# bastienjacquet/CudaDepthMapIntegration

Measured on AMD Instinct MI355X. Metric: Gvoxel-projections/s, higher is better.
Workload: dtype f64

## Files before the change

### cudadepthmapintegration_amd/build.py

```python
from __future__ import annotations

import os
import re
import shutil
import subprocess
from concurrent.futures import ThreadPoolExecutor

_HERE = os.path.dirname(os.path.abspath(__file__))
ROOT = os.path.dirname(_HERE)
CSRC = os.path.join(_HERE, "csrc")
OBJ_DIR = os.path.join(ROOT, "build", "obj")
LIB_PATH = os.path.join(CSRC, "libdmi_hip.so")

SOURCES = ["fusion_kernels.hip", "fusion_tile.hip", "fusion_classify.hip", "coloration_kernels.hip", "mesh_depth_render.hip", "grid_post.hip", "point_smooth.hip", "isosurface.hip", "isosurface_components.hip", "isosurface_smooth.hip", "isosurface_decimate.hip", "isosurface_holes.hip", "isosurface_support.hip", "depth_consistency.hip", "depth_speckle.hip", "scene_bounds.hip", "dmi_capi.hip", "dmi_capi_views.hip", "dmi_capi_fuse.hip", "dmi_capi_mesh.hip", "dmi_capi_color.hip", "dmi_capi_consistency.hip", "dmi_capi_speckle.hip", "dmi_capi_bounds.hip", "dmi_multi.hip", "host/recon_host.cpp", "host/vti_reader.cpp", "host/vtp_reader.cpp", "host/recon_cli.cpp", "host/color_cli.cpp", "host/dmi_host_capi.cpp"]
HEADERS = ["fusion_kernels.h", "view_records.h", "fusion_launch_rules.h", "fusion_device.h", "dmi_buffer.h", "dmi_context.h", "dmi_color_context.h", "coloration_kernels.h", "mesh_depth_render.h", "depth_consistency.h", "depth_speckle.h", "depth_speckle_rules.h", "union_find_device.h", "scene_bounds.h", "scene_bounds_rules.h", "point_smooth_rules.h", "rounded_quotient.h", "fusion_tile_acc.inc", "isosurface_table.inc", os.path.join("host", "recon_host.h"),
           os.path.join("host", "vtk_xml_data.h"), os.path.join("host", "vti_reader.h"), os.path.join("host", "vtp_reader.h"),
           os.path.join("host", "recon_cli.h"), os.path.join("host", "color_cli.h"), os.path.join("host", "fan_triangulate.h"),
           os.path.join("..", "..", "include", "dmi.h"), os.path.join("..", "..", "include", "dmi_host.h")]
CLI_MAINS = ["recon_cli_main.cpp", "color_cli_main.cpp"]

COMMON_FLAGS = ["-O3", "-std=c++17", "-fPIC", "-ffp-contract=off", "-fno-fast-math", "-Wall", "-Wno-unused-function",
                "-Wno-inline-asm", "-Wno-pass-failed"]
HIP_FLAGS = ["--offload-arch=gfx950", "-mllvm", "-disable-promote-alloca-to-vector", "-Xoffload-linker", "--discard-all"]
OPTIONAL_LLVM_FLAGS = ["-amdgpu-use-amdgpu-trackers=1"]


def _probe_llvm_flag(flag: str) -> bool:
    import tempfile
# ... 178 lines not shown
    for m in re.finditer(r"\.amdhsa_kernel (_ZN3dmi\S*fuse_tile_kernel\S*)\b(.*?)\.end_amdhsa_kernel", asm_text, re.S):
        size = re.search(r"\.amdhsa_private_segment_fixed_size (\d+)", m.group(2))
        out[m.group(1)] = int(size.group(1)) if size else 0
    return out


def lds_sizes(asm_text: str) -> dict:
    out = {}
    for m in re.finditer(r"\.amdhsa_kernel (_ZN3dmi\S*fuse_tile_kernel\S*)\b(.*?)\.end_amdhsa_kernel", asm_text, re.S):
        size = re.search(r"\.amdhsa_group_segment_fixed_size (\d+)", m.group(2))
        out[m.group(1)] = int(size.group(1)) if size else 0
    return out


def wait_state_counts(asm_text: str) -> dict:
    import re

    out = {}
    for m in re.finditer(r"^(_ZN3dmi\S*fuse_tile_kernel\S*):.*?\.end_amdhsa_kernel", asm_text, re.S | re.M):
        out[m.group(1)] = len(re.findall(r"^\s*s_nop\b", m.group(0), re.M))
    return out


def _audit_digest() -> str:
    return source_digest([os.path.join(CSRC, "fusion_tile.hip")] + _headers())


def audit_is_current() -> bool:
    import json

    marker = os.path.join(OBJ_DIR, "acc_audit.json")
    try:
        with open(marker) as fh:
            return json.load(fh).get("digest") == _audit_digest()
    except (OSError, ValueError):
        return False


def run_accumulator_audit(verbose: bool = False) -> int:
    import json
    import tempfile

    hipcc = hipcc_path()
    with tempfile.TemporaryDirectory() as tmp:
        out = os.path.join(tmp, "fusion_tile.s")
        cmd = [hipcc] + COMMON_FLAGS + HIP_FLAGS + ["--cuda-device-only", "-S", os.path.join(CSRC, "fusion_tile.hip"), "-o", out]
# ... 7 lines not shown
    nops = wait_state_counts(text)
    lds = lds_sizes(text)
    table = {}
    for name, size in scratch.items():
        m = re.search(r"fuse_tile_kernelI(\w)(\w)Li(\d+)ELi(\d)ELi(\d)ELi(\d)ELi(\d)ELb([01])ELb([01])ELb([01])ELb([01])ELb([01])(?:ELb([01]))?E", name)
        if not m:
            continue
        depth, grid, tk, wx, wy, minw, group, count, rot, genk, stay, win, zf = m.groups()
        key = f"depth={depth} grid={grid} tk={tk} waves={wx}x{wy} count={count} rot={rot} genk={genk} stay={stay} win={win} zf={zf or 0}"
        production = depth == "f" and count == "0" and genk == "0" and wx == "1" and wy == "1"
        limit = None if not production else ((16 if "-DDMI_TUNING" in COMMON_FLAGS else 0) if tk == "16" else 48)
        table[key] = {"scratch_bytes_per_lane": size, "production": production, "limit": limit, "s_nop": nops.get(name),
                      "lds_bytes_per_workgroup": lds.get(name, 0)}
        if limit is not None and size > limit:
            bad.append(f"{name}: {size} bytes of scratch memory per lane in a production instantiation (limit {limit})")
        waves_per_cu = 4 * (4 if tk == "16" else 5)
        if production and lds.get(name, 0) * waves_per_cu > 160 * 1024:
            bad.append(f"{name}: {lds[name]} bytes of LDS per one-wave workgroup: {waves_per_cu} of them do not fit a CU's 160 KB")
    if bad:
        raise RuntimeError("accumulator-register audit of fusion_tile.hip FAILED (a toolchain change broke the hidden "
                           "register file; results would be silently wrong):\n  " + "\n  ".join(bad[:20]))
    version = subprocess.run([hipcc, "--version"], capture_output=True, text=True).stdout.strip().splitlines()
    os.makedirs(OBJ_DIR, exist_ok=True)
    with open(os.path.join(OBJ_DIR, "acc_audit.json"), "w") as fh:
        json.dump({"instantiations": checked, "violations": 0, "hipcc": version[:2], "digest": _audit_digest(),
                   "scratch_bytes_per_lane": {"max": max(scratch.values()) if scratch else None,
                                              "instantiations_with_scratch": sum(1 for v in scratch.values() if v),
                                              "production_max": max([v["scratch_bytes_per_lane"] for v in table.values() if v["production"]] or [0])},
                   "instantiation_table": table}, fh, indent=1)
    if verbose:
        print(f"accumulator audit: {checked} fuse_tile_kernel instantiations clean ({version[0] if version else 'hipcc'})", flush=True)
    return checked


def _record(mode: str) -> None:
    import json
    import time

    try:
        os.makedirs(OBJ_DIR, exist_ok=True)
        with open(os.path.join(OBJ_DIR, "build_record.json"), "w") as fh:
            json.dump({"mode": mode, "library": os.path.relpath(LIB_PATH, ROOT), "digest": source_digest(), "time": time.time(),
                       "flags": COMMON_FLAGS + HIP_FLAGS}, fh)
    except OSError:
        pass


def build(force: bool = False, verbose: bool = False) -> str:
    if not force and not needs_build():
        _record("up_to_date: the library's digest file names the present sources and flags; nothing compiled")
        return LIB_PATH
    hipcc = hipcc_path()
    os.makedirs(OBJ_DIR, exist_ok=True)
    headers = _headers()
    digest = source_digest()
    if not force and os.path.exists(LIB_PATH) and os.path.exists(_digest_path()):
        srcs = [os.path.join(CSRC, s) for s in _sources()]
        if not any(_stale(_obj(s), [p] + headers) for s, p in zip(_sources(), srcs)):
            force = True

    def compile_one(src: str):
        path = os.path.join(CSRC, src)
        obj = _obj(src)
        if not force and not _stale(obj, [path] + headers):
            return
        cmd = [hipcc] + COMMON_FLAGS + (HIP_FLAGS if src.endswith(".hip") else []) + ["-c", path, "-o", obj]
        if verbose:
            print(" ".join(cmd), flush=True)
        subprocess.check_call(cmd)

    def audit_if_needed(_):
        if force or not audit_is_current():
            run_accumulator_audit(verbose)

    with ThreadPoolExecutor(max_workers=4) as ex:
        jobs = [ex.submit(compile_one, s) for s in _sources()] + [ex.submit(audit_if_needed, None)]
        for j in jobs:
            j.result()
    staged = os.path.join(OBJ_DIR, os.path.basename(LIB_PATH) + f".{os.getpid()}.tmp")
    cmd = [hipcc, "--offload-arch=gfx950", "-shared", "-fPIC"] + [_obj(s) for s in _sources()] + ["-lz", "-ldl", "-pthread", "-o", staged]
    if verbose:
        print(" ".join(cmd), flush=True)
    subprocess.check_call(cmd)
    os.replace(staged, LIB_PATH)
    with open(_digest_path(), "w") as fh:
        fh.write(digest + "\n")
    build_cli(verbose)
    build_color_cli(verbose)
    _record("rebuilt: hipcc compiled the stale objects and linked the library")
    return LIB_PATH


CLI_PATH = os.path.join(CSRC, "dmi_reconstruction")
COLOR_CLI_PATH = os.path.join(CSRC, "dmi_coloration")


def _link_tool(main_src: str, exe: str, verbose: bool) -> str:
    if os.path.basename(LIB_PATH) != "libdmi_hip.so" or LIB_OVERRIDE:
        return ""
# ... 26 lines not shown
```

### cudadepthmapintegration_amd/capi.py

```python
from __future__ import annotations

import ctypes
import os
import sys
from typing import NamedTuple

import numpy as np

from . import build as _build
from .scene import GridDesc, RayPotential, Views

DMI_OK = 0
DMI_F32, DMI_F64 = 0, 1
DMI_DEPTH_AUTO, DMI_DEPTH_F32, DMI_DEPTH_F64 = 0, 1, 2
DMI_COMPONENTS_MIN_TRIANGLES, DMI_COMPONENTS_LARGEST = 0, 1

VARIANT_EXACT_DIVISION = 1
VARIANT_GENERAL_K = 2
VARIANT_FORCE_GENERAL = 16
VARIANT_NO_BRICK_CLASSES = 256
VARIANT_KEEP_BEHIND_ADDS = 1024
VARIANT_NO_INTERIOR = 2048
VARIANT_XCD_RUNS = 8192
VARIANT_ZMAJOR_SLOTS = 16384
VARIANT_PERSISTENT_ALWAYS = 32768
VARIANT_PERSISTENT_NEVER = 65536
VARIANT_NO_WINDOWS = 262144
VARIANT_WINDOWS_ALWAYS = 524288
VARIANT_COST_ORDER = 1048576
VARIANT_NO_COST_ORDER = 2097152
VARIANT_BRICK_CLASSES_ALWAYS = 131072
VARIANT_FIXED_TILE_SHAPE = 4096
VARIANT_SPATIAL_ORDER = 512
VARIANT_TILE_SHAPE = {"tk16_w5_g8_1x1": 0, "tk8_w6_g8_2x2": 32, "tk16_w5_g8_2x2": 64, "tk8_w6": 96, "tk8_w7_g8": 128, "tk16_w5_g4": 160,
                      "tk16_w6_g2": 192, "tk8_w6_g8_1x1": 224}


class GridDescC(ctypes.Structure):
    _fields_ = [("cell_dims", ctypes.c_int32 * 3), ("origin", ctypes.c_double * 3),
                ("spacing", ctypes.c_double * 3), ("grid_matrix", ctypes.c_double * 16)]


class RayPotentialC(ctypes.Structure):
    _fields_ = [("thickness", ctypes.c_double), ("rho", ctypes.c_double), ("eta", ctypes.c_double),
                ("delta", ctypes.c_double)]


class OptionsC(ctypes.Structure):
    _fields_ = [("device", ctypes.c_int32), ("grid_dtype", ctypes.c_int32), ("depth_storage", ctypes.c_int32),
                ("count_hits", ctypes.c_int32), ("kernel_variant", ctypes.c_int32), ("z_first", ctypes.c_int32),
                ("stream", ctypes.c_void_p), ("external_grid", ctypes.c_void_p)]


# ... 1559 lines not shown
```

### cudadepthmapintegration_amd/csrc/dmi_capi_fuse.hip

```cpp
#include "dmi_context.h"

#include <algorithm>
#include <cmath>
#include <cstdlib>
#include <cstring>

using dmi::drain_events;
using dmi::EventPair;
using dmi::fail;
using dmi::flush_zero_fill;
using dmi::FuseArgs;
using dmi::FuseConfig;
using dmi::guarded;
using dmi::MapRec;
using dmi::TileArgs;
using dmi::TileMapRec;

namespace {

int sync_maps(dmi_context *ctx) {
  dmi_context::Views &v = ctx->views;
  const size_t n = v.h_maps.size();
  const size_t cap = std::max<size_t>(64, n * 2);
  bool fresh = false;
// ... 142 lines not shown
  if (!whole_grid) {
    t.sbz_first = a.k_first / (2 * sh.tk);
    t.super_z = (a.k_first + a.k_count + 2 * sh.tk - 1) / (2 * sh.tk) - t.sbz_first;
  }
  if (t.bricks_x > 2047 || t.bricks_y > 2047 || t.bricks_z > 1023)
    return fail(ctx, DMI_ERR_INVALID_ARGUMENT, "dmi_fuse: more bricks along an axis than the tiled kernel's order entries hold");
  t.slot_base = t.sbz_first * t.super_x * t.super_y * 32;
  t.slot_count = t.super_x * t.super_y * t.super_z * 32;
  const int rc = slot_permutation(ctx, t.super_x, t.super_y, t.super_z, (cfg.variant & dmi::VAR_ZMAJOR_SLOTS) != 0, &t.sb_perm);
  if (rc != DMI_OK) return rc;
  t.xcd_run_wg = 32 * std::max(1, t.super_x * t.super_y);
  if (((int64_t)t.super_x * t.super_y * t.super_z * 32 + 16 * (int64_t)t.xcd_run_wg + 64) > (int64_t)0x7fffffff)
    return fail(ctx, DMI_ERR_INVALID_ARGUMENT, "dmi_fuse: grid too large for one launch");
  t.depth_bytes = (int32_t)((int64_t)a.W * a.H * (ctx->views.depth_f64 ? 8 : 4));
  t.kz0 = a.kz0;
  t.ox = a.ox; t.oy = a.oy; t.oz = a.oz; t.sx = a.sx; t.sy = a.sy; t.sz = a.sz;
  std::memcpy(t.g, a.g, sizeof(t.g));
  t.thick = a.thick; t.delta = a.delta; t.rho_pos = a.rho_pos; t.rho_neg = a.rho_neg;
  t.slope = a.slope; t.free_space = a.free_space;
  t.tile_maps = ctx->views.tile_maps.as<TileMapRec>();
  t.grid = a.grid; t.voxel_hits = a.voxel_hits; t.map_hits = a.map_hits;
  t.rotated = dmi::grid_axis_aligned(ctx->grid) ? 0 : 1;
  t.flags = ((cfg.variant & dmi::VAR_NO_INTERIOR) ? dmi::TILE_FLAG_NO_INTERIOR : 0) |
            ((cfg.variant & dmi::VAR_XCD_RUNS) ? dmi::TILE_FLAG_XCD_RUNS : 0);
  t.maps = ctx->views.maps.as<MapRec>();
  t.wbricks_x = (a.nx + 7) / 8;
  t.wbricks_y = (a.ny + 7) / 8;
  return DMI_OK;
}

int cz_table(dmi_context *ctx, const FuseArgs &a, TileArgs *t) {
  const size_t table_doubles = std::max<size_t>(ctx->views.h_maps.size(), 4) * (size_t)t->kpad;
  const size_t need = table_doubles + (size_t)dmi::kFreeSumsMax + 1;
  const int rc = dmi::ensure_idle_buffer(ctx, ctx->tables.cz_table, need * 8, need * 2 * 8);
  if (rc != DMI_OK) return rc;
  t->cz_table = ctx->tables.cz_table.as<double>();
  if (!a.init_from_grid && !ctx->opt.count_hits && a.n_maps <= dmi::kFreeSumsMax) t->free_sums = t->cz_table + table_doubles;
  return DMI_OK;
}

int zero_row(dmi_context *ctx, TileArgs *t) {
  bool fresh = false;
  const int rc = dmi::ensure_idle_buffer(ctx, ctx->tables.zero_row, (uint64_t)t->class_pitch, (uint64_t)t->class_pitch, &fresh);
  if (rc != DMI_OK) return rc;
  if (fresh) DMI_HIP(ctx, hipMemsetAsync(ctx->tables.zero_row.ptr, dmi::BRICK_MIXED, (size_t)t->class_pitch, ctx->stream));
  t->classes = ctx->tables.zero_row.as<uint8_t>();
  t->class_pitch = 0;
// ... 300 lines not shown
```

### cudadepthmapintegration_amd/csrc/fusion_classify.hip

```cpp
#include <algorithm>
#include <cstring>

#include <stdlib.h>

#include "fusion_kernels.h"
#include "fusion_device.h"

namespace dmi {

namespace {

template <typename T>
__device__ __forceinline__ T cload(const T *p) {
  return *reinterpret_cast<const T __attribute__((address_space(4))) *>(reinterpret_cast<uintptr_t>(p));
}

__device__ __forceinline__ float float_below(double d) {
  float f = (float)d;
  if ((double)f > d) f = nextafterf(f, -__builtin_inff());
  return f;
}
__device__ __forceinline__ float float_above(double d) {
  float f = (float)d;
  if ((double)f < d) f = nextafterf(f, __builtin_inff());
// ... 409 lines not shown
  } else if (fp.partial) {
    cls = border_class<GK>(a, fp, pyramid_query<5>(maps[m].pyramid, P, fp.x0, fp.x1, fp.y0, fp.y1));
  }
  const bool inherit_mixed = cls == (uint8_t)(BRICK_MIXED | (MIXED_FREE_OR_NODEPTH << 2)) && speckled;
  coarse[(int64_t)((cbz * cy_n + cby) * cx_n + cbx) * a.class_pitch + m] = inherit_mixed ? (uint8_t)(cls | COARSE_CHILDREN_WRITTEN) : cls;
  if ((cls & 3) == BRICK_MIXED && !inherit_mixed) return;
  for (int dz = 0; dz < per_z; ++dz) {
    const int bz = bz0 + dz;
    if (bz >= bz_first + bz_count) break;
    for (int dy = 0; dy < 4; ++dy) {
      const int by = cby * 4 + dy;
      if (by >= a.wbricks_y) break;
      for (int dx = 0; dx < 4; ++dx) {
        const int bx = cbx * 4 + dx;
        if (bx >= a.wbricks_x) break;
        classes[(int64_t)((bz * a.wbricks_y + by) * a.wbricks_x + bx) * a.class_pitch + m] = cls;
      }
    }
  }
}

constexpr int kWindow = 16;

template <int kQueryTiles, int kChildren, bool ROT, bool GK>
__global__ __launch_bounds__(256) void classify_kernel(const TileArgs a, const MapRec *__restrict__ maps,
                                                       const PyramidDesc P, int tk, uint8_t *__restrict__ classes,
                                                       const uint8_t *__restrict__ coarse, int group_views) {
  constexpr int children = kChildren;
  constexpr int views_per_wave = 64 / children;
  constexpr int per_z = children / 16;
  __shared__ float2 window_mm[4 * views_per_wave][kWindow * kWindow];
  __shared__ uint8_t window_fl[4 * views_per_wave][kWindow * kWindow];
  const int bz_first = 2 * a.sbz_first;
  const int bz_count = min(2 * a.super_z, a.bricks_z - bz_first);
  const int cx_n = (a.wbricks_x + 3) / 4, cy_n = (a.wbricks_y + 3) / 4;
  const int lane = threadIdx.x & 63, wave = __builtin_amdgcn_readfirstlane(threadIdx.x >> 6);
  const int local = blockIdx.x;
  const int cbx = local % cx_n;
  const int ct = local / cx_n;
  const int cby = ct % cy_n, cbz = ct / cy_n + bz_first / per_z;
  const int chunk0 = blockIdx.y * group_views;
  const uint8_t *__restrict__ crow = coarse + (int64_t)((cbz * cy_n + cby) * cx_n + cbx) * a.class_pitch + a.first_map + chunk0;
  const unsigned long long unproven = __builtin_amdgcn_ballot_w64(
      lane < group_views && chunk0 + lane < a.n_maps && (crow[lane] & (3 | COARSE_CHILDREN_WRITTEN)) == BRICK_MIXED);
  if (unproven == 0) return;
  unsigned long long items = views_per_wave == 1 ? unproven & (0x1111111111111111ull << wave)
                                                 : (unproven | (unproven >> 1)) & (0x0101010101010101ull << (2 * wave));
  const int child = lane % children;
  const int bx = cbx * 4 + (child & 3), by = cby * 4 + ((child >> 2) & 3), bz = cbz * per_z + (child >> 4);
  const bool in_grid = bx < a.wbricks_x && by < a.wbricks_y && bz < bz_first + bz_count;
  uint8_t *__restrict__ out = classes + (int64_t)((bz * a.wbricks_y + by) * a.wbricks_x + bx) * a.class_pitch;
  while (items) {
    const int first = __builtin_ctzll(items);
    items &= items - 1;
    const int rel = first + lane / children;
    const int mm = chunk0 + rel;
    const int m = a.first_map + min(mm, a.n_maps - 1);
    const bool mine = in_grid && ((unproven >> rel) & 1ull);
    const MapRec *__restrict__ mr = maps + m;
    BoxFootprint fp;
    fp.query = false;
    fp.partial = false;
    fp.in_margin = false;
    fp.cls = BRICK_SKIP;
// ... 60 lines not shown
            TileAcc d;
            for (int ty = ty0; ty <= ty1; ++ty)
              for (int tx = tx0; tx <= tx1; ++tx) {
                const int w = (ty - wy0) * kWindow + (tx - wx0);
                const float2 mm = win_mm[w];
                d.add_tile(DepthTile{mm.x, mm.y, (uint32_t)win_fl[w], 0u});
              }
            cls = fp.partial ? border_class<GK>(a, fp, d) : class_from_bounds(a, d, fp.czmin, fp.czmax);
            from_window = true;
          }
          __builtin_amdgcn_fence(__ATOMIC_RELEASE, "wavefront");
          __builtin_amdgcn_wave_barrier();
        }
      }
    }
    if (query && !from_window) {
      const TileAcc d = pyramid_query<kQueryTiles>(mr->pyramid, P, fp.x0, fp.x1, fp.y0, fp.y1);
      cls = fp.partial ? border_class<GK>(a, fp, d) : class_from_bounds(a, d, fp.czmin, fp.czmax);
    }
    if (mine) out[m] = cls;
  }
}

constexpr int kOriginViews = 8;
#ifdef DMI_WINPAIR_BRICK_MAJOR
constexpr int kOriginBricks = 256, kOriginWaveSets = 1, kOriginAlign = 4;
#else
constexpr int kOriginBricks = 64, kOriginWaveSets = 4, kOriginAlign = kWinPairBlockViews;
static_assert(kOriginViews * kOriginWaveSets == kWinPairBlockViews, "a workgroup's views are one block of the pair table");
#endif
constexpr uint32_t kNotWanted = 0xfffffffeu;
template <bool ROT>
__global__ __launch_bounds__(256) void window_origin_kernel(const TileArgs a, const MapRec *__restrict__ maps, int tk,
                                                            uint8_t *__restrict__ classes, WinPair *__restrict__ origins,
                                                            int group_views) {
  __shared__ WinPair tile[kOriginViews * kOriginWaveSets][kOriginBricks + 1];
#ifdef DMI_WINPAIR_BRICK_MAJOR
  __shared__ int64_t rows[256];
#endif
  const int bz_first = 2 * a.sbz_first;
  const int bz_count = min(2 * a.super_z, a.bricks_z - bz_first);
  const int64_t n_bricks = (int64_t)a.wbricks_x * a.wbricks_y * bz_count;
  const int lane = threadIdx.x & 63;
  const int tb = threadIdx.x % kOriginBricks;
  const int wset = kOriginWaveSets > 1 ? __builtin_amdgcn_readfirstlane(threadIdx.x / kOriginBricks) : 0;
  const int64_t local = (int64_t)blockIdx.x * kOriginBricks + tb;
  const bool exists = local < n_bricks;
  const int bx = (int)(local % a.wbricks_x);
  const int64_t t = local / a.wbricks_x;
  const int by = (int)(t % a.wbricks_y), bz = (int)(t / a.wbricks_y) + bz_first;
  const int64_t row = (((int64_t)bz * a.wbricks_y + by) * a.wbricks_x + bx) * a.class_pitch;
  const bool eligible = exists && bz * tk + tk <= a.nz;
  (void)lane;
  double wxa, wya, wza;
  {
    const double gx = a.ox + (bx * 8 + 0.5) * a.sx;
    const double gy = a.oy + (by * 8 + 0.5) * a.sy;
    const double gz = a.oz + ((bz * tk + a.kz0) + 0.5) * a.sz;
    wxa = row4(a.g + 0, gx, gy, gz), wya = row4(a.g + 4, gx, gy, gz), wza = row4(a.g + 8, gx, gy, gz);
  }
  const int m_begin = a.first_map, m_end = a.first_map + a.n_maps;
  const int g_wg = (m_begin & ~(kOriginAlign - 1)) + blockIdx.y * (group_views * kOriginWaveSets);
  const int slot0 = wset * group_views;
  const int g_lo = g_wg + slot0;
#ifdef DMI_WINPAIR_BRICK_MAJOR
  rows[threadIdx.x] = row;
#endif
  uint32_t held[kOriginViews / 4];
#pragma unroll
  for (int g = 0; g < kOriginViews / 4; ++g) {
    const int m4 = g_lo + 4 * g;
    held[g] = (eligible && 4 * g < group_views && m4 < m_end) ? *reinterpret_cast<const uint32_t *>(classes + row + m4) : 0u;
    if (4 * g < group_views) {
#pragma unroll
      for (int q = 0; q < 4; ++q) tile[slot0 + 4 * g + q][tb].origin = kNotWanted;
    }
  }
#pragma unroll
  for (int g = 0; g < kOriginViews / 4; ++g) {
    const int m4 = g_lo + 4 * g;
    if (4 * g >= group_views || m4 >= m_end) break;
    const uint32_t c4 = held[g];
#pragma unroll 1
    for (int q = 0; q < 4; ++q) {
      const int m = m4 + q;
      const uint8_t c = (uint8_t)(c4 >> (8 * q));
      const bool want = eligible && m >= m_begin && m < m_end && (c & 0x1f) == (uint8_t)(BRICK_MIXED | (MIXED_FREE_OR_NODEPTH << 2));
      if (__builtin_amdgcn_ballot_w64(want) == 0) continue;
      WinPair wp;
      wp.origin = kNotWanted;
      wp.ax = wp.ay = wp.acz = 0.f;
      if (cload(&a.win_recs[m].e_abs) < __builtin_inff()) {
        const MapRec *src = maps + m;
        const TileMapRec *tsrc = a.tile_maps + m;
        const FootRec *fr = a.foot_recs + m;
        const float(*scp)[4] = tk == 16 ? fr->s16 : fr->s8;
        if (want) {
          const double cza = ((cload(&src->rt[8]) * wxa + cload(&src->rt[9]) * wya) + cload(&src->rt[10]) * wza) + cload(&src->rt[11]);
          const double hxa = __builtin_fma(cload(&tsrc->cpx), wxa, __builtin_fma(cload(&tsrc->cpy), wya, __builtin_fma(cload(&tsrc->cpz), wza, cload(&tsrc->cp0))));
          const double hya = __builtin_fma(cload(&tsrc->cqx), wxa, __builtin_fma(cload(&tsrc->cqy), wya, __builtin_fma(cload(&tsrc->cqz), wza, cload(&tsrc->cq0))));
          const float hx0 = (float)hxa, hy0 = (float)hya, z0 = (float)cza;
          float umin = __builtin_inff(), umax = -__builtin_inff(), vmin = __builtin_inff(), vmax = -__builtin_inff();
// ... 15 lines not shown
            const int cxc = a.W / 2, cyc = a.H / 2;
            const int x0 = (int)__builtin_ceilf(umin - 0.5f - e) + cxc, x1 = (int)__builtin_floorf(umax + 0.5f + e) + cxc;
            const int y0 = (int)__builtin_ceilf(vmin - 0.5f - e) + cyc, y1 = (int)__builtin_floorf(vmax + 0.5f + e) + cyc;
            if (x0 >= -kValidMargin && y0 >= -kValidMargin && x1 < a.W + kValidMargin && y1 < a.H + kValidMargin &&
                x1 - x0 < kWindowCols && y1 - y0 < kWindowRows) {
              wp.origin = (uint32_t)(x0 + kValidMargin) | ((uint32_t)(y0 + kValidMargin) << 16);
              wp.ax = (float)(hxa - (double)(x0 + kWinAnchorX - cxc) * cza);
              wp.ay = (float)(hya - (double)(y0 + kWinAnchorY - cyc) * cza);
              wp.acz = z0;
            }
          }
        }
      }
      if (want) {
        if (wp.origin != kNotWanted)
          tile[slot0 + 4 * g + q][tb] = wp;
        else
          classes[row + m] = (uint8_t)(c | CLASS_NO_WINDOW);
      }
    }
  }
  __syncthreads();
#ifdef DMI_WINPAIR_BRICK_MAJOR
  const int v = threadIdx.x & (kOriginViews - 1);
  const int m = g_lo + v;
  if (v < group_views && m < m_end) {
#pragma unroll
    for (int it = 0; it < 8; ++it) {
      const int b = (threadIdx.x >> 3) + 32 * it;
      const WinPair wp = tile[v][b];
      if (wp.origin != kNotWanted) origins[rows[b] + m] = wp;
    }
  }
#else
  const int wg_views = group_views * kOriginWaveSets;
  const int lg = 31 - __builtin_clz((unsigned)wg_views);
  const int64_t brick0 = (int64_t)blockIdx.x * kOriginBricks + (int64_t)bz_first * a.wbricks_y * a.wbricks_x;
  for (int e = threadIdx.x; e < kOriginBricks * wg_views; e += 256) {
    const int b = e >> lg, v = e & (wg_views - 1);
    const int m = g_wg + v;
    if (m >= m_end) continue;
    const WinPair wp = tile[v][b];
    if (wp.origin != kNotWanted) origins[win_pair_index(brick0 + b, m, a.n_class_bricks)] = wp;
  }
#endif
}


__device__ __forceinline__ bool slot_to_brick(const TileArgs &a, int slot, int &bx, int &by, int &bz) {
  const int within = slot & 31;
  const int code = a.sb_perm[(slot - a.slot_base) >> 5];
  const int sbx = code & 1023, sby = (code >> 10) & 1023, sbz = (code >> 20) + a.sbz_first;
  bx = sbx * 4 + (within & 3);
  by = sby * 4 + ((within >> 2) & 3);
  bz = sbz * 2 + (within >> 4);
  return bx < a.bricks_x && by < a.bricks_y && bz < a.bricks_z;
}

constexpr int kWorkLevels = 4;

__global__ __launch_bounds__(256) void brick_work_kernel(const TileArgs a, int wx, int wy, int n_slots,
// ... 290 lines not shown
      DMI_UPLOAD(double, float);
  } else {
    if (out_is_f64)
      DMI_UPLOAD(float, double);
    else
      DMI_UPLOAD(float, float);
  }
#undef DMI_UPLOAD
  return hipGetLastError();
}

hipError_t launch_build_pyramid_levels(int64_t n_maps, const PyramidDesc &P, DepthTile *pyramids, hipStream_t stream) {
  if (n_maps <= 0 || P.n_levels <= 1) return hipSuccess;
  hipLaunchKernelGGL(pyramid_levels_kernel, dim3((unsigned)n_maps), dim3(1024), 0, stream, P, pyramids);
  return hipGetLastError();
}

hipError_t launch_window_origins(const TileArgs &a, const MapRec *maps_dev, int tk, uint8_t *classes, int general_k,
                                 hipStream_t stream) {
  if (general_k || !a.win_origin || a.n_maps <= 0) return hipSuccess;
  const int bz_count = std::min(2 * a.super_z, a.bricks_z - 2 * a.sbz_first);
  const int64_t n_bricks = (int64_t)a.wbricks_x * a.wbricks_y * bz_count;
  if (n_bricks <= 0) return hipSuccess;
  const int64_t brick_groups = (n_bricks + kOriginBricks - 1) / kOriginBricks;
  const int span = a.first_map + a.n_maps - (a.first_map & ~(kOriginAlign - 1));
  int group_views = kOriginViews;
  const auto view_groups = [&](int gv) { return (span + gv * kOriginWaveSets - 1) / (gv * kOriginWaveSets); };
  while (group_views > 4 && brick_groups * view_groups(group_views) < 2048) group_views >>= 1;
  if (brick_groups > (int64_t)0x7fffffff || a.n_class_bricks > (int64_t)0x7fffffff) return hipErrorInvalidConfiguration;
  const dim3 grid((unsigned)brick_groups, (unsigned)view_groups(group_views));
  if (a.rotated)
    hipLaunchKernelGGL((window_origin_kernel<true>), grid, dim3(256), 0, stream, a, maps_dev, tk, classes, a.win_origin, group_views);
  else
    hipLaunchKernelGGL((window_origin_kernel<false>), grid, dim3(256), 0, stream, a, maps_dev, tk, classes, a.win_origin, group_views);
  return hipGetLastError();
}

hipError_t launch_classify_bricks(const TileArgs &a, const MapRec *maps_dev, const PyramidDesc &P, int tk, uint8_t *classes,
                                  uint8_t *coarse, int general_k, hipStream_t stream) {
  const int bz_count = std::min(2 * a.super_z, a.bricks_z - 2 * a.sbz_first);
  const int64_t n_bricks = (int64_t)a.wbricks_x * a.wbricks_y * bz_count;
  if (n_bricks <= 0 || a.n_maps <= 0) return hipSuccess;
  if (n_bricks > (int64_t)0x7fffffff || (a.n_maps + 3) / 4 > 65535) return hipErrorInvalidConfiguration;
  const int per_z = 32 / tk;
  const int64_t n_boxes = (int64_t)((a.wbricks_x + 3) / 4) * ((a.wbricks_y + 3) / 4) * ((bz_count + per_z - 1) / per_z);
  const dim3 coarse_grid((unsigned)((n_boxes + 3) / 4), (unsigned)((a.n_maps + 63) / 64));
#define DMI_LAUNCH_COARSE(R, G) \
  hipLaunchKernelGGL((classify_coarse_kernel<R, G>), coarse_grid, dim3(64, 4), 0, stream, a, maps_dev, P, tk, classes, coarse)
  if (a.rotated && general_k)
    DMI_LAUNCH_COARSE(true, true);
  else if (a.rotated)
    DMI_LAUNCH_COARSE(true, false);
  else if (general_k)
    DMI_LAUNCH_COARSE(false, true);
  else
    DMI_LAUNCH_COARSE(false, false);
#undef DMI_LAUNCH_COARSE
  hipError_t e = hipGetLastError();
  if (e != hipSuccess) return e;
  int group_views = 64;
  while (group_views > 8 && n_boxes * ((a.n_maps + group_views - 1) / group_views) < 2048) group_views >>= 1;
  const dim3 fine_grid((unsigned)n_boxes, (unsigned)((a.n_maps + group_views - 1) / group_views));
  [[maybe_unused]] int q = 5;
#ifdef DMI_TUNING
  if (const char *env = getenv("DMI_QUERY_TILES")) q = atoi(env);
#endif
  const bool wide = tk == 8;
#define DMI_LAUNCH_FINE_G(Q, C, R, G) \
  hipLaunchKernelGGL((classify_kernel<Q, C, R, G>), fine_grid, dim3(256), 0, stream, a, maps_dev, P, tk, classes, coarse, group_views)
#define DMI_LAUNCH_FINE_R(Q, C, R)      \
  do {                                  \
    if (general_k)                      \
      DMI_LAUNCH_FINE_G(Q, C, R, true); \
    else                                \
      DMI_LAUNCH_FINE_G(Q, C, R, false);\
  } while (0)
#define DMI_LAUNCH_FINE(Q)                      \
  do {                                          \
    if (wide && a.rotated)                      \
      DMI_LAUNCH_FINE_R(Q, 64, true);           \
    else if (wide)                              \
      DMI_LAUNCH_FINE_R(Q, 64, false);          \
    else if (a.rotated)                         \
      DMI_LAUNCH_FINE_R(Q, 32, true);           \
    else                                        \
// ... 52 lines not shown
```

### cudadepthmapintegration_amd/csrc/fusion_kernels.h

```cpp
#pragma once

#include <hip/hip_runtime.h>
#include <stddef.h>
#include <stdint.h>
#include <string.h>

#include "fusion_launch_rules.h"
#include "point_smooth_rules.h"
#include "view_records.h"

struct dmi_context;

namespace dmi {

int grid_pointer_for_sums(::dmi_context *ctx, void **ptr);

struct alignas(16) DepthTile {
  float dmin, dmax;
  uint32_t flags;
  uint32_t pad;
};
enum TileFlags : uint32_t { TILE_HAS_SENTINEL = 1, TILE_HAS_VALID = 2, TILE_HAS_NAN = 4, TILE_PART_HOLE_FREE = 8, TILE_PART_NO_VALID = 16 };
constexpr uint8_t COARSE_CHILDREN_WRITTEN = 0x80;

// ... 70 lines not shown
  const double *free_sums;
  const int32_t *sb_perm;
  unsigned long long *wg_times;
  int64_t wg_times_n;
  int32_t *queue_heads;
  WinPair *win_origin;
  int64_t n_class_bricks;
  const WinRec *win_recs;
  const FootRec *foot_recs;
  int32_t vb_bytes, vb_rowskip;
  int32_t win_cx, win_cy;
};
constexpr int kFreeSumsMax = 4096;
__host__ __device__ inline int32_t pack_brick(int bx, int by, int bz) { return (int32_t)((uint32_t)bx | ((uint32_t)by << 11) | ((uint32_t)bz << 22)); }
static_assert(offsetof(TileArgs, nx) == 0 && offsetof(TileArgs, nz) == 8 && offsetof(TileArgs, kpad) == 32 &&
                  offsetof(TileArgs, bricks_x) == 36 && offsetof(TileArgs, bricks_z) == 44 && offsetof(TileArgs, sbz_first) == 60,
              "TileArgs head layout");
enum TileKernelFlags : int32_t {
  TILE_FLAG_NO_INTERIOR = 1,
  TILE_FLAG_XCD_RUNS = 2,
  TILE_FLAG_COST_ORDER = 4,
  TILE_FLAG_DBG_SKIP_WINDOW_PAIRS = 256,
  TILE_FLAG_DBG_ONLY_WINDOW_PAIRS = 512,
  TILE_FLAG_DBG_NO_WINDOW_LOADS = 1024
};

enum BrickClass : uint8_t {
  BRICK_MIXED = 0,
  BRICK_FREE = 1,
  BRICK_BEHIND = 2,
  BRICK_SKIP = 3
};

enum MixedReason : uint8_t {
  MIXED_UNSPECIFIED = 0,
  MIXED_DEGENERATE = 1,
  MIXED_CAMERA_PLANE = 2,
  MIXED_IMAGE_BORDER = 3,
  MIXED_NAN_DEPTH = 4,
  MIXED_SENTINEL_AND_DEPTH = 5,
  MIXED_NEAR_SURFACE = 6,
  MIXED_FREE_OR_NODEPTH = 7
};

struct FuseConfig {
  int depth_is_f64;
  int grid_is_f64;
// ... 209 lines not shown
```

### cudadepthmapintegration_amd/csrc/fusion_launch_rules.h

```cpp
#pragma once
#include <stddef.h>
#include <stdint.h>

namespace dmi {

constexpr int64_t kNoClassesMaxBricks = 1024;
constexpr int kNoClassesMaxViews = 48;

enum VariantBits : int {
  VAR_EXACT_DIVISION = 1,
  VAR_GENERAL_K = 2,
  VAR_BLOCK_SHAPE_MASK = 12,
  VAR_FORCE_GENERAL = 16,
  VAR_TILE_SHAPE_MASK = 0xE0,
  VAR_TILE_SHAPE_SHIFT = 5,
  VAR_NO_BRICK_CLASSES = 256,
  VAR_SPATIAL_ORDER = 512,
  VAR_FIXED_TILE_SHAPE = 4096,
  VAR_KEEP_BEHIND_ADDS = 1024,
  VAR_NO_INTERIOR = 2048,
  VAR_XCD_RUNS = 8192,
  VAR_ZMAJOR_SLOTS = 16384,
  VAR_PERSISTENT_ALWAYS = 32768,
  VAR_PERSISTENT_NEVER = 65536,
  VAR_BRICK_CLASSES_ALWAYS = 131072,
  VAR_NO_WINDOWS = 262144,
  VAR_WINDOWS_ALWAYS = 524288,
  VAR_COST_ORDER = 1048576,
  VAR_NO_COST_ORDER = 2097152
};

constexpr int kCostOrderMaxSlots = 0;

struct HoleTraits {
  bool scattered = false;
  bool holes = false;
  bool tall_by_holes = false;
  bool many_borders = false;
  bool mostly_empty = false;
};

inline HoleTraits hole_traits(unsigned long long mingled, unsigned long long without, unsigned long long strips, unsigned long long pixels) {
  HoleTraits h;
  h.scattered = without <= 6 * mingled;
  h.holes = h.scattered && mingled * 160 > strips;
  h.tall_by_holes = h.scattered && mingled * 80 > strips;
  h.many_borders = mingled * 25 > strips;
  h.tall_by_holes = h.tall_by_holes || h.many_borders;
  if (!h.holes) h.mostly_empty = without * 4 >= pixels && pixels > 0;
  return h;
}

// ... 22 lines not shown
#else
#define DMI_RULES_HD
#endif
constexpr int kWinPairBlockViews = 32;
DMI_RULES_HD inline int64_t win_pair_index(int64_t brick, int32_t view, int64_t n_class_bricks) {
  return (((int64_t)(view >> 5) * n_class_bricks + brick) << 5) + (view & 31);
}

inline bool win_pair_pieces_addressable(int64_t n_class_bricks) { return n_class_bricks < (int64_t(1) << 22); }
struct WinPairFill {
  uint64_t first;
  uint32_t range;
};
DMI_RULES_HD inline uint64_t win_pair_piece_stride(uint64_t n_class_bricks) { return n_class_bricks << 9; }
DMI_RULES_HD inline WinPairFill win_pair_fill(uint64_t brick, uint32_t block, uint64_t n_class_bricks, uint32_t class_pitch) {
  const uint64_t table_bytes = (n_class_bricks * class_pitch) << 4;
  WinPairFill f;
  f.first = (n_class_bricks * block + brick) << 9;
  const uint64_t rest = table_bytes > f.first ? table_bytes - f.first : 0;
  f.range = rest > 0xffffffffull ? 0xffffffffu : (uint32_t)rest;
  return f;
}

inline bool zero_free(bool init_from_grid, bool grid_free_of_negative_zero, bool count_hits, int variant) {
  return (!init_from_grid || grid_free_of_negative_zero) && !count_hits && !(variant & VAR_KEEP_BEHIND_ADDS);
}

struct WindowsQuestion {
  bool tier1;
  bool general_k;
  bool count_hits;
  int variant;
  bool holes, many_borders;
  bool any_tier1;
  bool zero_free;
  bool depth_f64;
};
inline bool use_windows(const WindowsQuestion &q) {
  return q.tier1 && !q.general_k && !q.count_hits && !(q.variant & (VAR_NO_WINDOWS | VAR_NO_INTERIOR)) &&
         (q.holes || q.many_borders || (q.variant & VAR_WINDOWS_ALWAYS)) && q.any_tier1 && q.zero_free && !q.depth_f64;
}

inline bool cost_order(int waves_per_workgroup, int variant, size_t n_slots) {
  return waves_per_workgroup == 1 && !(variant & VAR_NO_COST_ORDER) && ((variant & VAR_COST_ORDER) || n_slots <= (size_t)kCostOrderMaxSlots);
}

// ... 2 lines not shown
```

Measured before the change: 3115.

## Reshape window-origin workgroups into templated view/wave-set forms with occupancy-driven selection

```diff
diff --git a/cudadepthmapintegration_amd/build.py b/cudadepthmapintegration_amd/build.py
--- a/cudadepthmapintegration_amd/build.py
+++ b/cudadepthmapintegration_amd/build.py
@@ -4,6 +4,7 @@
 import re
 import shutil
 import subprocess
+import threading
 from concurrent.futures import ThreadPoolExecutor
 
 _HERE = os.path.dirname(os.path.abspath(__file__))
@@ -228,6 +229,81 @@
     return out
 
 
+PREP_KERNELS = ("classify_coarse_kernel", "classify_kernel", "window_origin_kernel")
+
+
+def prep_kernel_table(asm_text: str) -> dict:
+    out = {}
+    for m in re.finditer(r"^(_ZN3dmi\S*):[^\n]*$(.*?)^; Occupancy: (\d+)", asm_text, re.S | re.M):
+        name, body = m.group(1), m.group(2)
+        kernel = next((k for k in PREP_KERNELS if re.search(r"\d+" + k + "I", name)), None)
+        if kernel is None:
+            continue
+
+        def field(key):
+            f = re.search(r"^; " + key + r": (\d+)", body, re.M)
+            return int(f.group(1)) if f else 0
+
+        args = re.search(kernel + r"I((?:L[ib]\d+E)+)EEv", name)
+        key = kernel + "<" + ",".join(re.findall(r"L[ib](\d+)E", args.group(1) if args else "")) + ">"
+        meta = re.search(r"\.max_flat_workgroup_size:\s*(\d+)\s*\n\s*\.name:\s*" + re.escape(name) + r"\s", asm_text)
+        out[key] = {"vgprs": field("TotalNumVgprs"), "sgprs": field("TotalNumSgprs"), "lds_bytes_per_workgroup": field("LDSByteSize"),
+                    "scratch_bytes_per_lane": field("ScratchSize"), "threads_per_workgroup": int(meta.group(1)) if meta else None,
+                    "waves_per_simd": int(m.group(3))}
+    return out
+
+
+def run_prep_audit(verbose: bool = False) -> dict:
+    import json
+    import tempfile
+
+    with tempfile.TemporaryDirectory() as tmp:
+        out = os.path.join(tmp, "fusion_classify.s")
+        cmd = [hipcc_path()] + COMMON_FLAGS + HIP_FLAGS + ["--cuda-device-only", "-S", os.path.join(CSRC, "fusion_classify.hip"), "-o", out]
+        if verbose:
+            print(" ".join(cmd), flush=True)
+        subprocess.check_call(cmd)
+        with open(out) as fh:
+            table = prep_kernel_table(fh.read())
+    with _AUDIT_LOCK:
+        rec = _read_audit_record()
+        rec["preparation_kernels"] = table
+        rec["preparation_digest"] = _prep_audit_digest()
+        os.makedirs(OBJ_DIR, exist_ok=True)
+        with open(os.path.join(OBJ_DIR, "acc_audit.json"), "w") as fh:
+            json.dump(rec, fh, indent=1)
+    if verbose:
+        print(f"preparation kernels: {len(table)} instantiations recorded in acc_audit.json", flush=True)
+    return table
+
+
+_AUDIT_LOCK = threading.Lock()
+
+
+def _read_audit_record() -> dict:
+    import json
+
+    try:
+        with open(os.path.join(OBJ_DIR, "acc_audit.json")) as fh:
+            return json.load(fh)
+    except (OSError, ValueError):
+        return {}
+
+
+def _prep_audit_digest() -> str:
+    return source_digest([os.path.join(CSRC, "fusion_classify.hip")] + _headers())
+
+
+def prep_audit_is_current() -> bool:
+    import json
+
+    try:
+        with open(os.path.join(OBJ_DIR, "acc_audit.json")) as fh:
+            return json.load(fh).get("preparation_digest") == _prep_audit_digest()
+    except (OSError, ValueError):
+        return False
+
+
 def _audit_digest() -> str:
     return source_digest([os.path.join(CSRC, "fusion_tile.hip")] + _headers())
 
@@ -281,12 +357,14 @@
                            "register file; results would be silently wrong):\n  " + "\n  ".join(bad[:20]))
     version = subprocess.run([hipcc, "--version"], capture_output=True, text=True).stdout.strip().splitlines()
     os.makedirs(OBJ_DIR, exist_ok=True)
-    with open(os.path.join(OBJ_DIR, "acc_audit.json"), "w") as fh:
-        json.dump({"instantiations": checked, "violations": 0, "hipcc": version[:2], "digest": _audit_digest(),
-                   "scratch_bytes_per_lane": {"max": max(scratch.values()) if scratch else None,
-                                              "instantiations_with_scratch": sum(1 for v in scratch.values() if v),
-                                              "production_max": max([v["scratch_bytes_per_lane"] for v in table.values() if v["production"]] or [0])},
-                   "instantiation_table": table}, fh, indent=1)
+    with _AUDIT_LOCK:
+        kept = {k: v for k, v in _read_audit_record().items() if k.startswith("preparation_")}
+        with open(os.path.join(OBJ_DIR, "acc_audit.json"), "w") as fh:
+            json.dump({"instantiations": checked, "violations": 0, "hipcc": version[:2], "digest": _audit_digest(),
+                       "scratch_bytes_per_lane": {"max": max(scratch.values()) if scratch else None,
+                                                  "instantiations_with_scratch": sum(1 for v in scratch.values() if v),
+                                                  "production_max": max([v["scratch_bytes_per_lane"] for v in table.values() if v["production"]] or [0])},
+                       "instantiation_table": table, **kept}, fh, indent=1)
     if verbose:
         print(f"accumulator audit: {checked} fuse_tile_kernel instantiations clean ({version[0] if version else 'hipcc'})", flush=True)
     return checked
@@ -332,8 +410,12 @@
         if force or not audit_is_current():
             run_accumulator_audit(verbose)
 
+    def prep_audit_if_needed(_):
+        if force or not prep_audit_is_current():
+            run_prep_audit(verbose)
+
     with ThreadPoolExecutor(max_workers=4) as ex:
-        jobs = [ex.submit(compile_one, s) for s in _sources()] + [ex.submit(audit_if_needed, None)]
+        jobs = [ex.submit(compile_one, s) for s in _sources()] + [ex.submit(audit_if_needed, None), ex.submit(prep_audit_if_needed, None)]
         for j in jobs:
             j.result()
     staged = os.path.join(OBJ_DIR, os.path.basename(LIB_PATH) + f".{os.getpid()}.tmp")
diff --git a/cudadepthmapintegration_amd/capi.py b/cudadepthmapintegration_amd/capi.py
--- a/cudadepthmapintegration_amd/capi.py
+++ b/cudadepthmapintegration_amd/capi.py
@@ -29,6 +29,7 @@
 VARIANT_WINDOWS_ALWAYS = 524288
 VARIANT_COST_ORDER = 1048576
 VARIANT_NO_COST_ORDER = 2097152
+VARIANT_PREP_LARGE_FORMS = 4194304
 VARIANT_BRICK_CLASSES_ALWAYS = 131072
 VARIANT_FIXED_TILE_SHAPE = 4096
 VARIANT_SPATIAL_ORDER = 512
diff --git a/cudadepthmapintegration_amd/csrc/dmi_capi_fuse.hip b/cudadepthmapintegration_amd/csrc/dmi_capi_fuse.hip
--- a/cudadepthmapintegration_amd/csrc/dmi_capi_fuse.hip
+++ b/cudadepthmapintegration_amd/csrc/dmi_capi_fuse.hip
@@ -188,7 +188,8 @@
   t.grid = a.grid; t.voxel_hits = a.voxel_hits; t.map_hits = a.map_hits;
   t.rotated = dmi::grid_axis_aligned(ctx->grid) ? 0 : 1;
   t.flags = ((cfg.variant & dmi::VAR_NO_INTERIOR) ? dmi::TILE_FLAG_NO_INTERIOR : 0) |
-            ((cfg.variant & dmi::VAR_XCD_RUNS) ? dmi::TILE_FLAG_XCD_RUNS : 0);
+            ((cfg.variant & dmi::VAR_XCD_RUNS) ? dmi::TILE_FLAG_XCD_RUNS : 0) |
+            ((cfg.variant & dmi::VAR_PREP_LARGE_FORMS) ? dmi::TILE_FLAG_PREP_LARGE_FORMS : 0);
   t.maps = ctx->views.maps.as<MapRec>();
   t.wbricks_x = (a.nx + 7) / 8;
   t.wbricks_y = (a.ny + 7) / 8;
diff --git a/cudadepthmapintegration_amd/csrc/fusion_classify.hip b/cudadepthmapintegration_amd/csrc/fusion_classify.hip
--- a/cudadepthmapintegration_amd/csrc/fusion_classify.hip
+++ b/cudadepthmapintegration_amd/csrc/fusion_classify.hip
@@ -455,8 +455,13 @@
 
 constexpr int kWindow = 16;
 
+#ifdef DMI_CLASSIFY_WAVES
+#define DMI_CLASSIFY_WAVES_ATTR __attribute__((amdgpu_waves_per_eu(DMI_CLASSIFY_WAVES, DMI_CLASSIFY_WAVES)))
+#else
+#define DMI_CLASSIFY_WAVES_ATTR
+#endif
 template <int kQueryTiles, int kChildren, bool ROT, bool GK>
-__global__ __launch_bounds__(256) void classify_kernel(const TileArgs a, const MapRec *__restrict__ maps,
+__global__ __launch_bounds__(256) DMI_CLASSIFY_WAVES_ATTR void classify_kernel(const TileArgs a, const MapRec *__restrict__ maps,
                                                        const PyramidDesc P, int tk, uint8_t *__restrict__ classes,
                                                        const uint8_t *__restrict__ coarse, int group_views) {
   constexpr int children = kChildren;
@@ -472,7 +477,7 @@
   const int cbx = local % cx_n;
   const int ct = local / cx_n;
   const int cby = ct % cy_n, cbz = ct / cy_n + bz_first / per_z;
-  const int chunk0 = blockIdx.y * group_views;
+  const int chunk0 = classify_view(blockIdx.y, 0, group_views);
   const uint8_t *__restrict__ crow = coarse + (int64_t)((cbz * cy_n + cby) * cx_n + cbx) * a.class_pitch + a.first_map + chunk0;
   const unsigned long long unproven = __builtin_amdgcn_ballot_w64(
       lane < group_views && chunk0 + lane < a.n_maps && (crow[lane] & (3 | COARSE_CHILDREN_WRITTEN)) == BRICK_MIXED);
@@ -579,19 +584,18 @@
   }
 }
 
-constexpr int kOriginViews = 8;
 #ifdef DMI_WINPAIR_BRICK_MAJOR
-constexpr int kOriginBricks = 256, kOriginWaveSets = 1, kOriginAlign = 4;
+constexpr int kOriginWgBricks = 256, kOriginAlign = 4;
 #else
-constexpr int kOriginBricks = 64, kOriginWaveSets = 4, kOriginAlign = kWinPairBlockViews;
-static_assert(kOriginViews * kOriginWaveSets == kWinPairBlockViews, "a workgroup's views are one block of the pair table");
+constexpr int kOriginWgBricks = kOriginBricks;
 #endif
 constexpr uint32_t kNotWanted = 0xfffffffeu;
-template <bool ROT>
-__global__ __launch_bounds__(256) void window_origin_kernel(const TileArgs a, const MapRec *__restrict__ maps, int tk,
+template <bool ROT, int kViews, int kWaveSets>
+__global__ __launch_bounds__(64 * kWaveSets * (kOriginWgBricks / 64)) void window_origin_kernel(const TileArgs a, const MapRec *__restrict__ maps, int tk,
                                                             uint8_t *__restrict__ classes, WinPair *__restrict__ origins,
                                                             int group_views) {
-  __shared__ WinPair tile[kOriginViews * kOriginWaveSets][kOriginBricks + 1];
+  [[maybe_unused]] constexpr int kThreads = 64 * kWaveSets * (kOriginWgBricks / 64);
+  __shared__ WinPair tile[kViews * kWaveSets][kOriginWgBricks + 1];
 #ifdef DMI_WINPAIR_BRICK_MAJOR
   __shared__ int64_t rows[256];
 #endif
@@ -599,9 +603,9 @@
   const int bz_count = min(2 * a.super_z, a.bricks_z - bz_first);
   const int64_t n_bricks = (int64_t)a.wbricks_x * a.wbricks_y * bz_count;
   const int lane = threadIdx.x & 63;
-  const int tb = threadIdx.x % kOriginBricks;
-  const int wset = kOriginWaveSets > 1 ? __builtin_amdgcn_readfirstlane(threadIdx.x / kOriginBricks) : 0;
-  const int64_t local = (int64_t)blockIdx.x * kOriginBricks + tb;
+  const int tb = threadIdx.x % kOriginWgBricks;
+  const int wset = kWaveSets > 1 ? __builtin_amdgcn_readfirstlane(threadIdx.x / kOriginWgBricks) : 0;
+  const int64_t local = (int64_t)blockIdx.x * kOriginWgBricks + tb;
   const bool exists = local < n_bricks;
   const int bx = (int)(local % a.wbricks_x);
   const int64_t t = local / a.wbricks_x;
@@ -617,15 +621,19 @@
     wxa = row4(a.g + 0, gx, gy, gz), wya = row4(a.g + 4, gx, gy, gz), wza = row4(a.g + 8, gx, gy, gz);
   }
   const int m_begin = a.first_map, m_end = a.first_map + a.n_maps;
-  const int g_wg = (m_begin & ~(kOriginAlign - 1)) + blockIdx.y * (group_views * kOriginWaveSets);
-  const int slot0 = wset * group_views;
+#ifdef DMI_WINPAIR_BRICK_MAJOR
+  const int g_wg = (m_begin & ~(kOriginAlign - 1)) + blockIdx.y * (group_views * kWaveSets);
+#else
+  const int g_wg = origin_view(m_begin, blockIdx.y, 0, group_views * kWaveSets);
+#endif
+  const int slot0 = origin_tile_slot(wset, 0, group_views);
   const int g_lo = g_wg + slot0;
 #ifdef DMI_WINPAIR_BRICK_MAJOR
   rows[threadIdx.x] = row;
 #endif
-  uint32_t held[kOriginViews / 4];
-#pragma unroll
-  for (int g = 0; g < kOriginViews / 4; ++g) {
+  uint32_t held[kViews / 4];
+#pragma unroll
+  for (int g = 0; g < kViews / 4; ++g) {
     const int m4 = g_lo + 4 * g;
     held[g] = (eligible && 4 * g < group_views && m4 < m_end) ? *reinterpret_cast<const uint32_t *>(classes + row + m4) : 0u;
     if (4 * g < group_views) {
@@ -634,7 +642,7 @@
     }
   }
 #pragma unroll
-  for (int g = 0; g < kOriginViews / 4; ++g) {
+  for (int g = 0; g < kViews / 4; ++g) {
     const int m4 = g_lo + 4 * g;
     if (4 * g >= group_views || m4 >= m_end) break;
     const uint32_t c4 = held[g];
@@ -696,7 +704,7 @@
   }
   __syncthreads();
 #ifdef DMI_WINPAIR_BRICK_MAJOR
-  const int v = threadIdx.x & (kOriginViews - 1);
+  const int v = threadIdx.x & (kViews - 1);
   const int m = g_lo + v;
   if (v < group_views && m < m_end) {
 #pragma unroll
@@ -707,10 +715,10 @@
     }
   }
 #else
-  const int wg_views = group_views * kOriginWaveSets;
+  const int wg_views = group_views * kWaveSets;
   const int lg = 31 - __builtin_clz((unsigned)wg_views);
-  const int64_t brick0 = (int64_t)blockIdx.x * kOriginBricks + (int64_t)bz_first * a.wbricks_y * a.wbricks_x;
-  for (int e = threadIdx.x; e < kOriginBricks * wg_views; e += 256) {
+  const int64_t brick0 = (int64_t)blockIdx.x * kOriginWgBricks + (int64_t)bz_first * a.wbricks_y * a.wbricks_x;
+  for (int e = threadIdx.x; e < kOriginWgBricks * wg_views; e += kThreads) {
     const int b = e >> lg, v = e & (wg_views - 1);
     const int m = g_wg + v;
     if (m >= m_end) continue;
@@ -1047,17 +1055,46 @@
   const int bz_count = std::min(2 * a.super_z, a.bricks_z - 2 * a.sbz_first);
   const int64_t n_bricks = (int64_t)a.wbricks_x * a.wbricks_y * bz_count;
   if (n_bricks <= 0) return hipSuccess;
-  const int64_t brick_groups = (n_bricks + kOriginBricks - 1) / kOriginBricks;
+  const int variant = (a.flags & TILE_FLAG_PREP_LARGE_FORMS) ? (int)VAR_PREP_LARGE_FORMS : 0;
+#define DMI_LAUNCH_ORIGINS(V, S)                                                                                             \
+  do {                                                                                                                       \
+    if (a.rotated)                                                                                                           \
+      hipLaunchKernelGGL((window_origin_kernel<true, V, S>), grid, dim3(threads), 0, stream, a, maps_dev, tk, classes,       \
+                         a.win_origin, group_views);                                                                        \
+    else                                                                                                                     \
+      hipLaunchKernelGGL((window_origin_kernel<false, V, S>), grid, dim3(threads), 0, stream, a, maps_dev, tk, classes,      \
+                         a.win_origin, group_views);                                                                        \
+  } while (0)
+#ifdef DMI_WINPAIR_BRICK_MAJOR
+  const int64_t brick_groups = (n_bricks + kOriginWgBricks - 1) / kOriginWgBricks;
   const int span = a.first_map + a.n_maps - (a.first_map & ~(kOriginAlign - 1));
-  int group_views = kOriginViews;
-  const auto view_groups = [&](int gv) { return (span + gv * kOriginWaveSets - 1) / (gv * kOriginWaveSets); };
-  while (group_views > 4 && brick_groups * view_groups(group_views) < 2048) group_views >>= 1;
+  int group_views = 8;
+  const auto view_groups = [&](int gv) { return (span + gv - 1) / gv; };
+  while (group_views > 4 && !variant && brick_groups * view_groups(group_views) < kPrepFillWorkgroups) group_views >>= 1;
   if (brick_groups > (int64_t)0x7fffffff || a.n_class_bricks > (int64_t)0x7fffffff) return hipErrorInvalidConfiguration;
   const dim3 grid((unsigned)brick_groups, (unsigned)view_groups(group_views));
-  if (a.rotated)
-    hipLaunchKernelGGL((window_origin_kernel<true>), grid, dim3(256), 0, stream, a, maps_dev, tk, classes, a.win_origin, group_views);
+  const unsigned threads = 256;
+  DMI_LAUNCH_ORIGINS(8, 1);
+#else
+  const int64_t brick_groups = origin_brick_groups(n_bricks);
+  const OriginForm form = origin_form(brick_groups, a.first_map, a.n_maps, variant);
+  const int group_views = form.views_per_wave;
+  if (brick_groups > (int64_t)0x7fffffff || a.n_class_bricks > (int64_t)0x7fffffff) return hipErrorInvalidConfiguration;
+  const dim3 grid((unsigned)brick_groups, (unsigned)origin_view_groups(a.first_map, a.n_maps, form.wg_views()));
+  const unsigned threads = (unsigned)form.threads();
+#ifdef DMI_PREP_PARENT_FORMS
+  if (form.tile_views == 32 && form.wave_sets == 4 && form.views_per_wave <= 8)
+    DMI_LAUNCH_ORIGINS(8, 4);
+#else
+  if (form.tile_views == 32 && form.wave_sets == 8 && form.views_per_wave == 4)
+    DMI_LAUNCH_ORIGINS(4, 8);
+  else if (form.tile_views == 16 && form.wave_sets == 4 && form.views_per_wave == 4)
+    DMI_LAUNCH_ORIGINS(4, 4);
+#endif
   else
-    hipLaunchKernelGGL((window_origin_kernel<false>), grid, dim3(256), 0, stream, a, maps_dev, tk, classes, a.win_origin, group_views);
+    return hipErrorInvalidConfiguration;
+#endif
+#undef DMI_LAUNCH_ORIGINS
   return hipGetLastError();
 }
 
@@ -1083,9 +1120,8 @@
 #undef DMI_LAUNCH_COARSE
   hipError_t e = hipGetLastError();
   if (e != hipSuccess) return e;
-  int group_views = 64;
-  while (group_views > 8 && n_boxes * ((a.n_maps + group_views - 1) / group_views) < 2048) group_views >>= 1;
-  const dim3 fine_grid((unsigned)n_boxes, (unsigned)((a.n_maps + group_views - 1) / group_views));
+  const int group_views = classify_group_views(n_boxes, a.n_maps, (a.flags & TILE_FLAG_PREP_LARGE_FORMS) ? (int)VAR_PREP_LARGE_FORMS : 0);
+  const dim3 fine_grid((unsigned)n_boxes, (unsigned)classify_view_groups(a.n_maps, group_views));
   [[maybe_unused]] int q = 5;
 #ifdef DMI_TUNING
   if (const char *env = getenv("DMI_QUERY_TILES")) q = atoi(env);
diff --git a/cudadepthmapintegration_amd/csrc/fusion_kernels.h b/cudadepthmapintegration_amd/csrc/fusion_kernels.h
--- a/cudadepthmapintegration_amd/csrc/fusion_kernels.h
+++ b/cudadepthmapintegration_amd/csrc/fusion_kernels.h
@@ -116,7 +116,8 @@
   TILE_FLAG_COST_ORDER = 4,
   TILE_FLAG_DBG_SKIP_WINDOW_PAIRS = 256,
   TILE_FLAG_DBG_ONLY_WINDOW_PAIRS = 512,
-  TILE_FLAG_DBG_NO_WINDOW_LOADS = 1024
+  TILE_FLAG_DBG_NO_WINDOW_LOADS = 1024,
+  TILE_FLAG_PREP_LARGE_FORMS = 2048
 };
 
 enum BrickClass : uint8_t {
diff --git a/cudadepthmapintegration_amd/csrc/fusion_launch_rules.h b/cudadepthmapintegration_amd/csrc/fusion_launch_rules.h
--- a/cudadepthmapintegration_amd/csrc/fusion_launch_rules.h
+++ b/cudadepthmapintegration_amd/csrc/fusion_launch_rules.h
@@ -27,7 +27,8 @@
   VAR_NO_WINDOWS = 262144,
   VAR_WINDOWS_ALWAYS = 524288,
   VAR_COST_ORDER = 1048576,
-  VAR_NO_COST_ORDER = 2097152
+  VAR_NO_COST_ORDER = 2097152,
+  VAR_PREP_LARGE_FORMS = 4194304
 };
 
 constexpr int kCostOrderMaxSlots = 0;
@@ -96,6 +97,52 @@
   return f;
 }
 
+constexpr int64_t kPrepFillWorkgroups = 2048;
+
+inline int classify_group_views(int64_t n_boxes, int32_t n_maps, int variant) {
+  int group_views = 64;
+  if (variant & VAR_PREP_LARGE_FORMS) return group_views;
+  while (group_views > 8 && n_boxes * ((n_maps + group_views - 1) / group_views) < kPrepFillWorkgroups) group_views >>= 1;
+  return group_views;
+}
+inline int classify_view_groups(int32_t n_maps, int group_views) { return (n_maps + group_views - 1) / group_views; }
+DMI_RULES_HD inline int classify_view(int block_y, int lane, int group_views) { return block_y * group_views + lane; }
+
+constexpr int kOriginBricks = 64;
+struct OriginForm {
+  int views_per_wave;
+  int wave_sets;
+  int tile_views;
+  DMI_RULES_HD int wg_views() const { return views_per_wave * wave_sets; }
+  DMI_RULES_HD int threads() const { return 64 * wave_sets; }
+};
+inline int64_t origin_brick_groups(int64_t n_bricks) { return (n_bricks + kOriginBricks - 1) / kOriginBricks; }
+DMI_RULES_HD inline int origin_span_first(int32_t first_map) { return first_map & ~(kWinPairBlockViews - 1); }
+inline int origin_view_groups(int32_t first_map, int32_t n_maps, int wg_views) {
+  return (first_map + n_maps - origin_span_first(first_map) + wg_views - 1) / wg_views;
+}
+DMI_RULES_HD inline int origin_tile_slot(int wset, int slot, int views_per_wave) { return wset * views_per_wave + slot; }
+DMI_RULES_HD inline int origin_view(int32_t first_map, int block_y, int tile_slot, int wg_views) {
+  return origin_span_first(first_map) + block_y * wg_views + tile_slot;
+}
+inline OriginForm origin_form(int64_t brick_groups, int32_t first_map, int32_t n_maps, int variant) {
+#ifdef DMI_PREP_PARENT_FORMS
+  OriginForm f{8, 4, 32};
+  if (variant & VAR_PREP_LARGE_FORMS) return f;
+  while (f.views_per_wave > 4 && brick_groups * origin_view_groups(first_map, n_maps, f.wg_views()) < kPrepFillWorkgroups) f.views_per_wave >>= 1;
+  return f;
+#else
+  const OriginForm small{4, 4, 16};
+#ifdef DMI_PREP_ORIGIN_HALF_BLOCKS
+  const OriginForm large = small;
+#else
+  const OriginForm large{4, 8, 32};
+#endif
+  if (variant & VAR_PREP_LARGE_FORMS) return large;
+  return brick_groups * origin_view_groups(first_map, n_maps, large.wg_views()) < kPrepFillWorkgroups ? small : large;
+#endif
+}
+
 inline bool zero_free(bool init_from_grid, bool grid_free_of_negative_zero, bool count_hits, int variant) {
   return (!init_from_grid || grid_free_of_negative_zero) && !count_hits && !(variant & VAR_KEEP_BEHIND_ADDS);
 }
```

New measurement: 3134 (median of 6 runs). About the same (+0.6%).
